# Psy-Fer/SquiggleKit

Measured on AMD Instinct MI355X. Metric: reads/sec MotifSeq DTW (4k-sample read x 200-sample motif), higher is better.
Workload: dtype f64 results; u32 fixed-point screening

## Files before the change

include/squigglekit_hip.h:

```cpp
#ifndef SQUIGGLEKIT_HIP_H
#define SQUIGGLEKIT_HIP_H

#include <stddef.h>
#include <stdint.h>

#ifdef __cplusplus
extern "C" {
#endif

typedef enum sk_status {
    SK_OK              =  0,
    SK_ERR_INVALID     = -1,
    SK_ERR_NO_DEVICE   = -2,
    SK_ERR_HIP         = -3,
    SK_ERR_NOMEM       = -4,
    SK_ERR_UNSUPPORTED = -5,
    SK_ERR_OVERFLOW    = -6
} sk_status;

enum { SK_SCALE_MEDMAD = 0, SK_SCALE_ZSCALE = 1 };

enum {
    SK_FLAG_EMPTY      = 1,
    SK_FLAG_DEGENERATE = 2,
// ... 338 lines not shown
    int32_t        kind;
    const void    *data;
    const int64_t *off;
} sk_fmt_col;
void *sk_fmt_rows(int64_t nrows, int32_t ncols, const sk_fmt_col *cols, const uint8_t *skip, int32_t nthreads,
                  int64_t *out_len);
void  sk_fmt_free(void *p);
void  sk_ndtr(const double *z, double *out, int64_t n);

int64_t sk_blow5_index(const void *buf, int64_t len, int64_t first, int64_t *rec_off, int64_t *rec_size, int64_t cap);
int64_t sk_blow5_index_some(const void *buf, int64_t len, int64_t pos, int64_t max_rec, int64_t *rec_off,
                            int64_t *rec_size, int64_t *next_pos);
int sk_blow5_rows_i16(const void *buf, int64_t len, const int64_t *rec_off, const int64_t *rec_size, int64_t nrec,
                      int32_t comp, int64_t stride, int16_t *rows, int32_t *nsamp, char *ids, int32_t id_width, double *calib,
                      int32_t *flags, int32_t nthreads);

int sk_comm_unique_id(void *id128);
int sk_comm_init_rank(const void *id128, int nranks, int rank);
int sk_comm_init_all(const int *devices, int ndev);
int sk_comm_info(int *nranks, int *rank);
int sk_comm_allgather_dev(const void *d_send, void *d_recv, size_t bytes);
int sk_comm_allgather_host(const void *send, void *recv, size_t bytes);
int sk_comm_destroy(void);

int sk_tunables(char *buf, int cap);

int sk_last_kernel_ms(float *prep_ms, float *main_ms);
int sk_last_dtw_retries(void);
int sk_last_dtw_tier2(void);
int sk_last_dtw_guard(int32_t *out );
int sk_last_dtw_premise_violations(void);
int sk_last_dtw_audit_mismatches(void);
int sk_last_dtw_window_steps(uint64_t *out );
int sk_last_f64_retries(void);
int sk_last_dtw_clock(double *ghz);
int sk_last_dtw_profile(float *dist_ms, int *dist_launches, float *start_ms, int *start_launches,
                        int *reads_per_launch);
int sk_synth_squiggles_dev(int16_t *d_sig, int64_t stride, int32_t nreads, int32_t nsamples,
                           uint64_t seed, const double *motif, int32_t nmotif);
typedef struct sk_synth_opts {
    int64_t        row0;
    int32_t        hit_permille;
    int32_t        stretch_permille;
    int32_t        stretch;
    const int16_t *tmpl;
    int32_t        ntmpl;
    double         tmpl_noise;
} sk_synth_opts;
int sk_synth_variant_dev(int16_t *d_sig, int64_t stride, int32_t nreads, int32_t nsamples, uint64_t seed,
                         const double *motif, int32_t nmotif, const sk_synth_opts *o);
int sk_synth_pa_dev(const int16_t *d_raw, int64_t stride, int32_t nreads, int32_t nsamples,
                    double offset, double range, double digitisation, double *d_out, int64_t *d_off);

typedef enum sk_pull_mode { SK_PULL_RAW = 0, SK_PULL_PA = 1 } sk_pull_mode;
int sk_pull_text(const int16_t *sig, int64_t stride, const int32_t *len, int32_t nreads, const double *calib, int32_t mode,
                 const char *prefix, const int64_t *prefix_off, char *text, int64_t capacity, int64_t *total,
                 int64_t *line_off);
int sk_pull_text_dev(const int16_t *d_sig, int64_t stride, const int32_t *d_len, int32_t nreads, const double *d_cal2,
                     int32_t mode, const char *d_prefix, const int64_t *d_prefix_off, char *d_text, int64_t capacity,
                     int64_t *total, int64_t *d_line_off);

typedef struct sk_det_params {
    int32_t w_short, w_long;
    double  th_short, th_long, peak_height;
} sk_det_params;
typedef struct sk_det_event {
// ... 73 lines not shown
```

squigglekit_amd/_lib.py:

```python
import ctypes as C
import os
import subprocess
import threading

import numpy as np

_HERE = os.path.dirname(os.path.abspath(__file__))
SO_PATH = os.environ.get("SK_LIB_PATH") or os.path.join(_HERE, "libsquigglekit_hip.so")
CSRC = os.path.join(_HERE, "csrc")


class SquiggleKitError(RuntimeError):
    def __init__(self, code, msg):
        super().__init__("squigglekit_hip error %d: %s" % (code, msg))
        self.code = code


SK_OK, SK_ERR_INVALID, SK_ERR_NO_DEVICE, SK_ERR_HIP, SK_ERR_NOMEM, SK_ERR_UNSUPPORTED, SK_ERR_OVERFLOW = 0, -1, -2, -3, -4, -5, -6
SK_SCALE = {"medmad": 0, "zscale": 1}
SK_PULL_RAW, SK_PULL_PA = 0, 1
SK_FLAG_EMPTY, SK_FLAG_DEGENERATE, SK_FLAG_RECENTRE = 1, 2, 4
SK_FLAG_CALIBRATING = 8
SK_STREAM_MAX_CALIB, SK_STREAM_MAX_SLOTS, SK_STREAM_MAX_POINTS = 65536, 65536, 1024

# ... 277 lines not shown
    "sk_dtw_subsequence_batch": (C.c_int, [_vp, C.c_int32, _vp, _vp, C.c_int32, _vp]),
    "sk_dtw_subsequence": (C.c_int, [_vp, C.c_int32, _vp, C.c_int32, _dp, _i32p, _i32p, _vp]),
    "sk_dtw_subsequence_cref": (C.c_int, [_vp, C.c_int32, _vp, C.c_int32, _dp, _i32p, _i32p]),
    "sk_normalise_i16": (C.c_int, [_vp, C.c_int32, C.c_int32, C.c_int32, C.c_int32, _vp, _i32p]),
    "sk_normalise_f64": (C.c_int, [_vp, C.c_int32, C.c_int32, C.c_int32, C.c_int32, _vp, _i32p]),
    "sk_tsv_count_lines": (C.c_int64, [_vp, C.c_size_t]),
    "sk_tsv_count_tokens": (C.c_int, [_vp, C.c_size_t, C.c_int32, C.c_int64, _vp, C.c_int32]),
    "sk_tsv_parse": (C.c_int, [_vp, C.c_size_t, C.c_int32, C.c_int64, _vp, _vp, _vp, _vp, _vp, _vp, _vp,
                               C.c_int32]),
    "sk_tsv_parse_centi": (C.c_int, [_vp, C.c_size_t, C.c_int32, C.c_int64, _vp, _vp, _vp, _vp, _vp, _vp, _vp,
                                     C.c_int32]),
    "sk_tsv_parse_i16": (C.c_int, [_vp, C.c_size_t, C.c_int32, C.c_int64, C.c_int64, _vp, _vp, _vp, _vp, _vp, _vp, _vp,
                                   _vp, C.c_int32]),
    "sk_fmt_rows": (_vp, [C.c_int64, C.c_int32, _vp, _vp, C.c_int32, _i64p]),
    "sk_fmt_free": (None, [_vp]),
    "sk_ndtr": (None, [_vp, _vp, C.c_int64]),
    "sk_blow5_index": (C.c_int64, [_vp, C.c_int64, C.c_int64, _vp, _vp, C.c_int64]),
    "sk_blow5_index_some": (C.c_int64, [_vp, C.c_int64, C.c_int64, C.c_int64, _vp, _vp, _vp]),
    "sk_blow5_rows_i16": (C.c_int, [_vp, C.c_int64, _vp, _vp, C.c_int64, C.c_int32, C.c_int64, _vp, _vp, _vp, C.c_int32, _vp, _vp,
                                    C.c_int32]),
    "sk_comm_unique_id": (C.c_int, [_vp]),
    "sk_comm_init_rank": (C.c_int, [_vp, C.c_int, C.c_int]),
    "sk_comm_init_all": (C.c_int, [_i32p, C.c_int]),
    "sk_comm_info": (C.c_int, [_i32p, _i32p]),
    "sk_comm_allgather_dev": (C.c_int, [_vp, _vp, C.c_size_t]),
    "sk_comm_allgather_host": (C.c_int, [_vp, _vp, C.c_size_t]),
    "sk_comm_destroy": (C.c_int, []),
    "sk_tunables": (C.c_int, [C.c_char_p, C.c_int]),
    "sk_last_kernel_ms": (C.c_int, [C.POINTER(C.c_float), C.POINTER(C.c_float)]),
    "sk_last_dtw_retries": (C.c_int, []),
    "sk_last_dtw_tier2": (C.c_int, []),
    "sk_last_dtw_guard": (C.c_int, [_i32p]),
    "sk_last_dtw_window_steps": (C.c_int, [_vp]),
    "sk_last_dtw_premise_violations": (C.c_int, []),
    "sk_last_dtw_audit_mismatches": (C.c_int, []),
    "sk_last_f64_retries": (C.c_int, []),
    "sk_last_dtw_clock": (C.c_int, [_dp]),
    "sk_last_dtw_profile": (C.c_int, [C.POINTER(C.c_float), _i32p, C.POINTER(C.c_float), _i32p, _i32p]),
    "sk_synth_squiggles_dev": (C.c_int, [_vp, C.c_int64, C.c_int32, C.c_int32, C.c_uint64, _vp, C.c_int32]),
    "sk_synth_variant_dev": (C.c_int, [_vp, C.c_int64, C.c_int32, C.c_int32, C.c_uint64, _vp, C.c_int32, _vp]),
    "sk_synth_pa_dev": (C.c_int, [_vp, C.c_int64, C.c_int32, C.c_int32, C.c_double, C.c_double, C.c_double, _vp, _vp]),
    "sk_pull_text": (C.c_int, [_vp, C.c_int64, _vp, C.c_int32, _vp, C.c_int32, _vp, _vp, _vp, C.c_int64, _i64p, _vp]),
    "sk_segment_sweep_i16": (C.c_int, [_vp, C.c_int64, _vp, C.c_int32, _vp, C.c_int32, _vp, _vp]),
    "sk_segment_sweep_dev_i16": (C.c_int, [_vp, C.c_int64, _vp, C.c_int32, _vp, C.c_int32, _vp, _vp]),
    "sk_segment_sweep_f64": (C.c_int, [_vp, _vp, _vp, C.c_int32, _vp, C.c_int32, _vp, _vp]),
    "sk_pull_text_dev": (C.c_int, [_vp, C.c_int64, _vp, C.c_int32, _vp, C.c_int32, _vp, _vp, _vp, C.c_int64, _i64p, _vp]),
    "sk_detect_events_i16": (C.c_int, [_vp, C.c_int64, _vp, C.c_int32, C.POINTER(DetParams), _vp, _vp, C.c_int64]),
    "sk_detect_events_dev_i16": (C.c_int, [_vp, C.c_int64, _vp, C.c_int32, C.POINTER(DetParams), _vp, _vp, C.c_int64]),
    "sk_hmm_viterbi_i16": (C.c_int, [_vp, C.c_int64, _vp, C.c_int32, _vp, C.POINTER(HmmModel), C.c_int32, _vp]),
    "sk_hmm_viterbi_dev_i16": (C.c_int, [_vp, C.c_int64, _vp, C.c_int32, _vp, C.POINTER(HmmModel), C.c_int32, _vp]),
    "sk_hmm_viterbi_f64_len": (C.c_int, [_vp, _vp, C.c_int32, C.POINTER(HmmModel), C.c_int32, _vp]),
    "sk_hmm_segments_i16": (C.c_int, [_vp, C.c_int64, _vp, C.c_int32, _vp, C.POINTER(HmmModel), C.c_int32, _vp, _vp, _vp,
                                      C.c_int64]),
    "sk_hmm_segments_dev_i16": (C.c_int, [_vp, C.c_int64, _vp, C.c_int32, _vp, C.POINTER(HmmModel), C.c_int32, _vp, _vp, _vp,
                                          C.c_int64]),
    "sk_hmm_segments_f64_len": (C.c_int, [_vp, _vp, C.c_int32, C.POINTER(HmmModel), C.c_int32, _vp, _vp, _vp, C.c_int64]),
    "sk_stream_open": (C.c_int, [_vp, _vp, C.c_int32, C.POINTER(StreamParams), _i32p]),
    "sk_stream_push_i16": (C.c_int, [C.c_int32, _vp, C.c_int32, _vp, C.c_int64, _vp, _vp]),
    "sk_stream_push_dev_i16": (C.c_int, [C.c_int32, _vp, C.c_int32, _vp, C.c_int64, _vp, _vp]),
    "sk_stream_flush": (C.c_int, [C.c_int32, _vp, C.c_int32, _vp]),
    "sk_stream_reset": (C.c_int, [C.c_int32, _vp, C.c_int32, _vp, _vp]),
    "sk_stream_close": (C.c_int, [C.c_int32]),
}


def build(force=False):
# ... 109 lines not shown
```

squigglekit_amd/csrc/sk_runtime.hip:

```cpp
#include "sk_common.h"
#include <string>
#include <string.h>
#include <mutex>
#include <stdio.h>
#include <stdlib.h>
#include <string.h>

static thread_local char  g_err[512] = "";
static thread_local int   g_cur = -1;
static sk_ctx             g_ctx[SK_MAX_DEVICES];
static std::mutex         g_mu;
static std::recursive_mutex g_ctx_mu[SK_MAX_DEVICES];

int sk_fail(int code, const char *fmt, ...)
{
    va_list ap;
    va_start(ap, fmt);
    vsnprintf(g_err, sizeof g_err, fmt, ap);
    va_end(ap);
    return code;
}

sk_entry::sk_entry() : sk_entry(g_cur) {}

// ... 16 lines not shown
sk_entry::~sk_entry() { if (c) g_ctx_mu[c - g_ctx].unlock(); }

sk_ctx *sk_ctx_of(int device) { return (device >= 0 && device < SK_MAX_DEVICES) ? &g_ctx[device] : nullptr; }
int sk_bound_device(void) { return g_cur; }

int sk_reserve(sk_ctx *c, sk_buf *b, size_t bytes)
{
    (void)c;
    if (bytes <= b->cap) return SK_OK;
    if (b->p) { SK_HIP(hipFree(b->p)); b->p = nullptr; b->cap = 0; }
    size_t want = bytes + bytes / 8 + 256;
    hipError_t e = hipMalloc(&b->p, want);
    if (e != hipSuccess) {
        b->p = nullptr;
        return sk_fail(SK_ERR_NOMEM, "hipMalloc(%zu) failed: %s", want, hipGetErrorString(e));
    }
    b->cap = want;
    return SK_OK;
}

int sk_second_stream(sk_ctx *c)
{
    if (!c->stream2) {
        SK_HIP(hipStreamCreateWithFlags(&c->stream2, hipStreamNonBlocking));
        for (int i = 0; i < 9; i++) SK_HIP(hipEventCreateWithFlags(&c->ev_chunk[i], hipEventDisableTiming));
    }
    return SK_OK;
}

struct sk_tunable { const char *name, *test_values, *what; };
static const sk_tunable SK_TUNABLES[] = {
    {"SK_DTW_SCHEME",         "full exact2", "DTW scheme: full = one exact pass, exact2 = two exact passes (default: fixed-point screening + certified window)"},
    {"SK_DTW_QL",             "8 16 64",     "lanes per read of the screening scheme (default: by motif length and batch size)"},
    {"SK_DTW_NOFUSE",         "1",           "filter + medmad as their own kernel instead of the screening pass's prologue"},
    {"SK_DTW_FORCE_RETRY_PM", "100 1000",    "per-mille of reads sent through the exact retry whatever the window pass certified (sensitivity runs)"},
    {"SK_DTW_SPAN",           "150 300",     "look-back of the window pass in columns (one tier)"},
    {"SK_DTW_SPAN2",          "0 500",       "look-back of the window pass's second tier (0: none)"},
    {"SK_DTW_CK",             "64 256",      "steps between checkpoints of the screening pass (multiple of 64)"},
    {"SK_DTW_NOSORT",         "1",           "window passes take the reads in file order"},
    {"SK_DTW_SORT_MIN",       "1",           "window passes sort chunks of at least this many reads"},
    {"SK_DTW_NO_EARLY",       "1",           "no early exact retry beside the window passes"},
    {"SK_DTW_NO_SIBLINGS",    "1",           "reads whose candidate columns fall into two clusters take the exact pass (no second window)"},
    {"SK_DTW_NOGUARD",        "1",           "screening scheme without its run-time guard (premise test in the window pass, audit, gated exact fallback): A/B cost runs"},
    {"SK_DTW_AUDIT_PERIOD",   "0 1 64",      "the audit re-runs one read in this many with the exact pass (default 4096; 0: no audit)"},
    {"SK_DTW_HOLE",           "qerr1 fma64 fma64x", "tests: a known precision hole put back (E = 1; the fma sample image for float64 reads, with / without the image-error guard) -- the guard has to notice and the records must not change"},
    {"SK_DTW_SCRATCH_MB",     "8 64",        "checkpoint scratch budget in MB (small values force many chunks)"},
    {"SK_DTW_NO_SMALL",       "1",           "small batches keep the batch lane layout"},
    {"SK_DTW_SMALL_MAX",      "0 100000",    "largest batch that spreads a read over 64 lanes"},
    {"SK_PREP_BLOCK",         "1",           "medmad statistics by the workgroup-per-read kernel"},
    {"SK_PREP_ROUNDS",        "1 3",         "grid rounds of the persistent statistics kernels"},
    {"SK_PREP_PERCU",         "1 2",         "workgroups per CU of the persistent statistics kernels"},
    {"SK_SEG_OLD",            "1",           "segmenter: numpy-order statistics kernels for every read"},
    {"SK_SEG_DELTA_SCALE",    "1e13",        "segmenter: certification margin multiplier (large: every read takes the numpy-order redo)"},
    {"SK_SEG_PA_F64",         "1",           "segmenter, raw reads through the pA conversion: expand to float64 and take the float64 kernels instead of the raw-domain kernel"},
    {"SK_SEG_NO_WG",          "1",           "segmenter, reads of 4 097 .. 65 536 samples: the wavefront-per-read statistics kernel (two looks at a read) instead of the workgroup-per-read one"},
    {"SK_SEG_WG_ALL",         "1",           "segmenter: the workgroup-per-read statistics kernel for every row of 4 097 .. 65 536 samples (default: where it is faster)"},
    {"SK_SEG_OCC",            "7 8",         "segmenter statistics kernel: waves per SIMD the registers are sized for"},
    {"SK_SEG_CHUNKS",         "2 8",         "segmenter: chunks of a large batch (walk of one beside the statistics of the next)"},
    {"SK_WALK_GENERAL",       "1",           "segmenter walk: general step (corrector test live)"},
    {"SK_WALK_SYNC",          "1",           "segmenter walk: run hopping with the 64 lanes of a wavefront on the same word (k_seg_walk3)"},
    {"SK_WALK_OWNPASS",       "1",           "segmenter walk: finds the quiet stretches and anchors in a pass of its own instead of taking the statistics kernel's hints"},
    {"SK_WALK_NOJUMP",        "1",           "segmenter walk: every run is hopped through, no jumps between the stretches of quiet entries"},
    {"SK_WALK_NOWAVE",        "1",           "segmenter walk: a lane per read also for long rows / small batches (no wavefront-per-read walk)"},
    {"SK_WALK_WAVE_MAXREADS", "0 1000000",   "segmenter walk: batches of up to this many reads take the wavefront-per-read walk (default: 16384, 131072 for rows beyond 4 096 samples)"},
    {"SK_DRNA_STEP",          "1",           "dRNA_segmenter, both branches: the per-sample scans instead of the scans by runs / by transitions"},
    {"SK_ROLL_TWO_KERNELS",   "1",           "dRNA_segmenter rolling-mean branch: filter kernel + prefix sums through HBM instead of the one-look kernel (prefix sums in LDS)"},
// ... 267 lines not shown
    if (!(c->retry_dev && c->dtwcnt.p)) return SK_OK;
    if (hipMemcpyAsync(out, (const int32_t *)c->dtwcnt.p + 8, 8 * sizeof(int32_t), hipMemcpyDeviceToHost, c->stream) != hipSuccess ||
        hipStreamSynchronize(c->stream) != hipSuccess)
        return sk_fail(SK_ERR_HIP, "reading the guard counters failed");
    return SK_OK;
}

int sk_last_dtw_premise_violations(void)
{
    int32_t g[8];
    const int rc = sk_last_dtw_guard(g);
    return rc ? rc : g[0];
}

int sk_last_dtw_audit_mismatches(void)
{
    int32_t g[8];
    const int rc = sk_last_dtw_guard(g);
    return rc ? rc : g[2];
}

int sk_last_dtw_window_steps(uint64_t *out)
{
    SK_ENTER(c);
    if (!out) return sk_fail(SK_ERR_INVALID, "NULL pointer");
    out[0] = out[1] = 0;
    if (!(c->retry_dev && c->dtwcnt.p && c->dtwcnt.cap >= 128)) return SK_OK;
    if (hipMemcpyAsync(out, (const char *)c->dtwcnt.p + 64, 16, hipMemcpyDeviceToHost, c->stream) != hipSuccess ||
        hipStreamSynchronize(c->stream) != hipSuccess)
        return sk_fail(SK_ERR_HIP, "reading the window-step counters failed");
    return SK_OK;
}

int sk_last_dtw_tier2(void)
{
    SK_ENTER(c);
    if (!(c->retry_dev && c->dtwcnt.p)) return 0;
    int32_t n = 0;
    if (hipMemcpyAsync(&n, (const int32_t *)c->dtwcnt.p + 1, sizeof n, hipMemcpyDeviceToHost, c->stream) != hipSuccess ||
        hipStreamSynchronize(c->stream) != hipSuccess)
        return sk_fail(SK_ERR_HIP, "reading the second-tier count failed");
    return n;
}

}
```

squigglekit_amd/csrc/sk_sdtwq.hip:

```cpp
#include "sk_sdtw_dev.h"
#include "sk_prepw_dev.h"
#include <math.h>
#include <stdlib.h>
#include <string.h>
#include <vector>

#ifndef SK_SDTWQ_FEED
#define SK_SDTWQ_FEED 0
#define SK_SDTWQ_MAIN 1
#endif

namespace {

template <int R>
__device__ __forceinline__ void qcolumn(const unsigned (&old)[R], unsigned (&nw)[R], const unsigned (&xq)[R],
                                        unsigned yq, unsigned dg, unsigned up)
{
    constexpr int R4 = R & ~3;
#pragma unroll
    for (int k = 0; k < R4; k += 4) {
        asm("v_min3_u32 %0, %12, %4, %13\n\t"
            "v_sad_u32 %0, %8, %14, %0 clamp\n\t"
            "v_min3_u32 %1, %4, %5, %0\n\t"
            "v_sad_u32 %1, %9, %14, %1 clamp\n\t"
            "v_min3_u32 %2, %5, %6, %1\n\t"
            "v_sad_u32 %2, %10, %14, %2 clamp\n\t"
            "v_min3_u32 %3, %6, %7, %2\n\t"
            "v_sad_u32 %3, %11, %14, %3 clamp"
            : "=&v"(nw[k]), "=&v"(nw[k + 1]), "=&v"(nw[k + 2]), "=&v"(nw[k + 3])
            : "v"(old[k]), "v"(old[k + 1]), "v"(old[k + 2]), "v"(old[k + 3]),
              "v"(xq[k]), "v"(xq[k + 1]), "v"(xq[k + 2]), "v"(xq[k + 3]),
              "v"(dg), "v"(up), "v"(yq));
        dg = old[k + 3];
        up = nw[k + 3];
    }
#pragma unroll
    for (int k = R4; k < R; k++) {
        asm("v_min3_u32 %0, %3, %1, %4\n\t"
            "v_sad_u32 %0, %2, %5, %0 clamp"
            : "=&v"(nw[k])
            : "v"(old[k]), "v"(xq[k]), "v"(dg), "v"(up), "v"(yq));
        dg = old[k];
        up = nw[k];
    }
}

__device__ __forceinline__ unsigned qimg(double v)
{
    return (unsigned)((int)rint(v * QSCALE)) + 0x80000000u;
}

template <int L>
__device__ __forceinline__ unsigned shr0(unsigned v, unsigned notfirst)
{
    if constexpr (L >= 16) {
        (void)notfirst;
        return (unsigned)__builtin_amdgcn_update_dpp(0, (int)v, (L == 16) ? DPP_ROW_SHR1 : DPP_WAVE_SHR1, 0xF, 0xF, true);
    } else {
        unsigned r;
        asm("s_nop 1\n\t"
            "v_and_b32_dpp %0, %1, %2 row_shr:1 row_mask:0xf bank_mask:0xf bound_ctrl:0"
            : "=v"(r) : "v"(v), "v"(notfirst));
        return r;
    }
}

struct wrec {
    int32_t tbase;
    int32_t jlo, jhi;
    int32_t flags;
};
struct sibrec {
    int32_t r;
    int32_t jlo, jhi;
    int32_t pad;
};

template <int L>
// ... 596 lines not shown
        const unsigned bq = (unsigned)a.qflag[r - a.read0];
        const double u = bestD * QSCALE, e = (double)a.qerr;
        const double e2 = (rec.flags & 4) ? 3.0 * e : e;
        const bool ok = fabs(u - (double)lq) <= e && u <= (double)bq + e2;
        if (!ok) { atomicAdd(&a.guard[SK_GUARD_VIOL], 1); atomicAdd(&a.guard[SK_GUARD_ALARM], 1); }
        return ok;
    };
    if (live && l == L - 1) {
        sk_hit h;
        h.n = n; h.flags = flags;
        const bool forced = a.force_retry && (((unsigned)r * 2654435761u) >> 22) < (unsigned)a.force_retry;
        bool certified = false;
        if (a.tier2 == 2) {
            h.dist = best; h.start = bestS; h.end = bestJ;
            h.n = (n > 0 && screened && bestS >= 0 && !forced && premise_holds(best, bestJ)) ? 1 : 0;
            a.sib_out[slot] = h;
        } else if (n <= 0) {
            h.dist = __builtin_nan(""); h.start = -1; h.end = -1;
            a.out[r] = h;
        } else if (screened && bestS >= 0 && !forced && (certified = premise_holds(best, bestJ))) {
            h.dist = best; h.start = bestS; h.end = bestJ;
            a.out[r] = h;
        } else if (!screened && a.early_cnt && !a.tier2) {
        } else {
            h.dist = __builtin_nan(""); h.start = -1; h.end = -1;
            a.out[r] = h;
            const bool violated = screened && bestS >= 0 && !forced && !certified;
            if (screened && a.soft && !forced && !violated) a.soft[atomicAdd(a.soft_cnt, 1)] = r;
            else                                            a.retry[atomicAdd(a.retry_cnt, 1)] = r;
        }
    }
}

typedef void (*sdtw_fn)(const sdtw_kargs);

template <int L, int FEED, int WHICH>
sdtw_fn pick_r(int R)
{
#define SK_KERNEL(RR) (WHICH == 0 ? (sdtw_fn)k_sdtw_q<L, RR, FEED, false> :     \
                       WHICH == 3 ? (sdtw_fn)k_sdtw_q<L, RR, FEED, (RR >= 2)> : \
                       WHICH == 1 ? (sdtw_fn)k_sdtw_p<L, RR, FEED> : (sdtw_fn)k_sdtw_w<L, RR, FEED>)
    switch (R) { SK_R_CASES_1_16(SK_KERNEL) }
    if constexpr (L != 64) {
        switch (R) { SK_R_CASES_17_32(SK_KERNEL) }
    }
#undef SK_KERNEL
    return nullptr;
}

template <int WHICH, int FEED>
sdtw_fn pick_l(int L, int R)
{
    if (L == 8)  return pick_r<8, FEED, WHICH>(R);
    if (L == 16) return pick_r<16, FEED, WHICH>(R);
    return pick_r<64, FEED, WHICH>(R);
}

}

#if SK_SDTWQ_FEED == 0
void *sk_sdtwq_pick_feed0(int which, int L, int R)
#elif SK_SDTWQ_FEED == 1
void *sk_sdtwq_pick_feed1(int which, int L, int R)
#else
void *sk_sdtwq_pick_feed2(int which, int L, int R)
#endif
{
    switch (which) {
    case 0: return (void *)pick_l<0, SK_SDTWQ_FEED>(L, R);
    case 1: return (void *)pick_l<1, SK_SDTWQ_FEED>(L, R);
    case 3: return (void *)pick_l<3, SK_SDTWQ_FEED>(L, R);
    default: return (void *)pick_l<2, SK_SDTWQ_FEED>(L, R);
    }
}

#ifdef SK_SDTWQ_MAIN
void *sk_sdtwq_pick_feed1(int which, int L, int R);
void *sk_sdtwq_pick_feed2(int which, int L, int R);

static void screen_layout(int N, int64_t nreads, int64_t maxlen, int *L, int *R)
{
    int l = (N <= 8 * 32 && nreads >= (maxlen > 8192 ? 65536 : 49152)) ? 8 : (N <= 16 * 32) ? 16 : 64;
    if (const char *e = sk_tune("SK_DTW_QL")) {
        const int v = atoi(e);
        if ((v == 8 && N <= 8 * 32) || (v == 16 && N <= 16 * 32) || v == 64) l = v;
    }
    *L = l;
    *R = (N + l - 1) / l;
}

constexpr int ORDER_BINS = 1024;

struct order_args {
    const wrec    *rec;
    const int32_t *qflag;
    int nreads, read0, span, ck, nck, L, wmax;
    int32_t *hist;
    int32_t *order;
};

__device__ __forceinline__ int order_key(const order_args &a, int i)
{
    const wrec q = a.rec[i];
    const unsigned b = (unsigned)a.qflag[i];
// ... 117 lines not shown
    int64_t chunk;
    while (true) {
        chunk = sk_dtw_chunk_reads(per_read, a->nreads);
        rc = sk_reserve(c, &c->ckpt, (size_t)chunk * (size_t)(nck > 0 ? nck : 1) * ck_bytes);
        if (!rc) rc = sk_reserve(c, &c->lastq, (size_t)chunk * lq_stride * sizeof(unsigned));
        if (!rc) rc = sk_reserve(c, &c->wstate, (size_t)chunk * state_bytes);
        if (!rc) rc = sk_reserve(c, &c->lsum, (size_t)chunk * (size_t)(nck + 1) * L * sizeof(unsigned));
        if (rc != SK_ERR_NOMEM || chunk <= 1024) break;
        sk_dtw_scratch_shrink(0);
    }
    if (rc) return rc;
    if ((rc = sk_reserve(c, &c->qflag, (size_t)chunk * sizeof(int32_t)))) return rc;
    if ((rc = sk_reserve(c, &c->wrec, (size_t)chunk * sizeof(wrec)))) return rc;
    if ((rc = sk_reserve(c, &c->wrecq, (size_t)chunk * sizeof(wrec)))) return rc;
    int sort_min = 32768;
    if (const char *e = sk_tune("SK_DTW_SORT_MIN")) { const int v = atoi(e); if (v > 0) sort_min = v; }
    const bool sorted = chunk >= sort_min && sk_tune("SK_DTW_NOSORT") == nullptr;
    if (sorted && (rc = sk_reserve(c, &c->order, ((size_t)chunk + ORDER_BINS) * sizeof(int32_t)))) return rc;
    const bool tiers = span2 > span;
    if (tiers && (rc = sk_reserve(c, &c->wsoft, ((size_t)chunk + 1) * sizeof(int32_t)))) return rc;
    const bool siblings = sk_tune("SK_DTW_NO_SIBLINGS") == nullptr;
    const int sib_cap = (int)(chunk / 64 + 1024);
    if (siblings) {
        if ((rc = sk_reserve(c, &c->sib, 16 + (size_t)sib_cap * sizeof(sibrec)))) return rc;
        if ((rc = sk_reserve(c, &c->sibout, (size_t)sib_cap * sizeof(sk_hit)))) return rc;
        if ((rc = sk_reserve(c, &c->sibstate, (size_t)sib_cap * (state_bytes + sizeof(wrec))))) return rc;
        if (c->stream3 && !c->ev_s[0])
            for (int i = 0; i < 2; i++) SK_HIP(hipEventCreateWithFlags(&c->ev_s[i], hipEventDisableTiming));
    }

    typedef void *(*pick_fn)(int, int, int);
    const pick_fn pk = a->feed == SK_FEED_I16 ? (pick_fn)sk_sdtwq_pick_feed0
                     : a->feed == SK_FEED_F64_NORM ? (pick_fn)sk_sdtwq_pick_feed1 : (pick_fn)sk_sdtwq_pick_feed2;
    sdtw_fn fq = (sdtw_fn)pk(P == 0 ? 3 : 0, L, R), fp = (sdtw_fn)pk(1, L, R), fw = (sdtw_fn)pk(2, L, R);
    if (!fq || !fp || !fw) return sk_fail(SK_ERR_UNSUPPORTED, "no screening kernel for L=%d R=%d", L, R);

    sdtw_kargs k = kargs_of(a);
    k.xlay = (const double *)c->motifw.p; k.xlayq = (const unsigned *)c->motifq.p; k.P = P; k.out = a->out;
    k.nck = nck; k.ck = ck; k.span = span; k.retry = d_retry; k.retry_cnt = d_retry_cnt;
    k.ckq = (unsigned *)c->ckpt.p; k.lastq = (unsigned *)c->lastq.p; k.lq_stride = (int64_t)lq_stride;
    k.qflag = (int32_t *)c->qflag.p; k.lsum = (unsigned *)c->lsum.p;
    k.wstate = (unsigned *)c->wstate.p; k.wrec = c->wrec.p; k.wrec_q = c->wrecq.p;
    k.early_cnt = d_early_cnt; k.early = d_early;
    k.qerr = (unsigned)(N + maxlen + 2);
    k.wmax = 4 * ck;
    k.lds_wave_words = (64 / L) * ck;
    k.guard = sk_tune("SK_DTW_NOGUARD") ? nullptr : (int32_t *)c->dtwcnt.p + 8;
    k.wsteps = (unsigned long long *)((char *)c->dtwcnt.p + 64);
    if (const char *e = sk_tune("SK_DTW_HOLE")) {
        k.hole = strcmp(e, "qerr1") == 0 ? SK_HOLE_QERR1 : strcmp(e, "fma64") == 0 ? SK_HOLE_FMA64
               : strcmp(e, "fma64x") == 0 ? SK_HOLE_FMA64_UNGUARDED : SK_HOLE_NONE;
        if (k.hole == SK_HOLE_QERR1) k.qerr = 1;
    }
    if (const char *e = sk_tune("SK_DTW_FORCE_RETRY_PM")) {
        const int pm = atoi(e);
        if (pm > 0) k.force_retry = pm >= 1000 ? 1024 : (pm * 1024 + 999) / 1000;
    }

    size_t fz_lds = 0;
    const sk_prep_fuse fz = a->fuse ? *a->fuse : sk_prep_fuse();
    if (a->fuse) {
        const int need = fz.mode == SK_PREP_ZSCALE ? (int)((a->stride * 2 + 15) / 16 * 4) : (((fz.hi - fz.lo - 1) + 3) & ~3);
        if (need > k.lds_wave_words) k.lds_wave_words = need;
    }
    fz_lds = (size_t)4 * (size_t)k.lds_wave_words * sizeof(unsigned);
    if (fz_lds + 5 * 1024 > 64 * 1024)
        return sk_fail(SK_ERR_INVALID, "SK_DTW_CK=%d with %d lanes per read needs %zu bytes of LDS per workgroup (limit 65536): "
// ... 97 lines not shown
```

Measured before the change: 16.82 million.

## Add hand-scheduled inline-asm window DTW kernel with LDS motif prefetch ring

Adds k_sdtw_wl, a new default exact window-pass kernel whose DTW cell update is written as interleaved inline GCN assembly (two cells in flight, f64 min/compare/cndmask for the start index). For R>16 it keeps the motif in LDS and software-prefetches the next four values with ds_read into a ring buffer while the current group computes. The intent is to beat the compiler's schedule on the serial dependency chain and cut register pressure. The old C++ kernel stays reachable through SK_DTW_WCELL=c, and a debug accessor for window records is added. Hand-written asm plus manual lgkmcnt waits risk hazards and make the code harder to maintain.

```diff
diff --git a/include/squigglekit_hip.h b/include/squigglekit_hip.h
--- a/include/squigglekit_hip.h
+++ b/include/squigglekit_hip.h
@@ -394,6 +394,7 @@
 int sk_last_dtw_premise_violations(void);
 int sk_last_dtw_audit_mismatches(void);
 int sk_last_dtw_window_steps(uint64_t *out );
+int sk_last_dtw_windows(int32_t *out , int nslots);
 int sk_last_f64_retries(void);
 int sk_last_dtw_clock(double *ghz);
 int sk_last_dtw_profile(float *dist_ms, int *dist_launches, float *start_ms, int *start_launches,
diff --git a/squigglekit_amd/_lib.py b/squigglekit_amd/_lib.py
--- a/squigglekit_amd/_lib.py
+++ b/squigglekit_amd/_lib.py
@@ -333,6 +333,7 @@
     "sk_last_dtw_tier2": (C.c_int, []),
     "sk_last_dtw_guard": (C.c_int, [_i32p]),
     "sk_last_dtw_window_steps": (C.c_int, [_vp]),
+    "sk_last_dtw_windows": (C.c_int, [_vp, C.c_int]),
     "sk_last_dtw_premise_violations": (C.c_int, []),
     "sk_last_dtw_audit_mismatches": (C.c_int, []),
     "sk_last_f64_retries": (C.c_int, []),
diff --git a/squigglekit_amd/csrc/sk_runtime.hip b/squigglekit_amd/csrc/sk_runtime.hip
--- a/squigglekit_amd/csrc/sk_runtime.hip
+++ b/squigglekit_amd/csrc/sk_runtime.hip
@@ -72,6 +72,7 @@
 static const sk_tunable SK_TUNABLES[] = {
     {"SK_DTW_SCHEME",         "full exact2", "DTW scheme: full = one exact pass, exact2 = two exact passes (default: fixed-point screening + certified window)"},
     {"SK_DTW_QL",             "8 16 64",     "lanes per read of the screening scheme (default: by motif length and batch size)"},
+    {"SK_DTW_WCELL",          "c",           "exact window pass with the cell as the compiler schedules it from C++ (k_sdtw_w) instead of the laid-out one (k_sdtw_wl)"},
     {"SK_DTW_NOFUSE",         "1",           "filter + medmad as their own kernel instead of the screening pass's prologue"},
     {"SK_DTW_FORCE_RETRY_PM", "100 1000",    "per-mille of reads sent through the exact retry whatever the window pass certified (sensitivity runs)"},
     {"SK_DTW_SPAN",           "150 300",     "look-back of the window pass in columns (one tier)"},
@@ -405,6 +406,19 @@
     return SK_OK;
 }
 
+int sk_last_dtw_windows(int32_t *out, int nslots)
+{
+    SK_ENTER(c);
+    if (!out || nslots < 0) return sk_fail(SK_ERR_INVALID, "NULL pointer or negative count");
+    const size_t bytes = (size_t)nslots * 4 * sizeof(int32_t);
+    if (!c->wrec.p || c->wrec.cap < bytes) return sk_fail(SK_ERR_INVALID, "no window records for %d slots", nslots);
+    if (bytes == 0) return SK_OK;
+    if (hipMemcpyAsync(out, c->wrec.p, bytes, hipMemcpyDeviceToHost, c->stream) != hipSuccess ||
+        hipStreamSynchronize(c->stream) != hipSuccess)
+        return sk_fail(SK_ERR_HIP, "reading the window records failed");
+    return SK_OK;
+}
+
 int sk_last_dtw_tier2(void)
 {
     SK_ENTER(c);
diff --git a/squigglekit_amd/csrc/sk_sdtwq.hip b/squigglekit_amd/csrc/sk_sdtwq.hip
--- a/squigglekit_amd/csrc/sk_sdtwq.hip
+++ b/squigglekit_amd/csrc/sk_sdtwq.hip
@@ -44,6 +44,131 @@
         up = nw[k];
     }
 }
+
+#define SK_W_A(m, c, t, dk, dkm1, sk, skm1, xk)                 \
+    "v_cmp_lt_f64 vcc, " dk ", " dkm1 "\n\t"                    \
+    "v_min_f64 " m ", " dk ", " dkm1 "\n\t"                     \
+    "v_add_f64 " c ", " xk ", -%[y]\n\t"                        \
+    "v_cndmask_b32 " t ", " skm1 ", " sk ", vcc\n\t"
+#define SK_W_B(m, c, t, dk, sk, u, us)                          \
+    "v_cmp_lt_f64 vcc, " u ", " m "\n\t"                        \
+    "v_min_f64 " m ", " u ", " m "\n\t"                         \
+    "v_add_f64 " dk ", |" c "|, " m "\n\t"                      \
+    "v_cndmask_b32 " sk ", " t ", " us ", vcc\n\t"
+#define SK_W_FOUR                                                                           \
+    SK_W_A("%[mb]", "%[cb]", "%[tb]", "%[d1]", "%[d0]", "%[s1]", "%[s0]", "%[x1]")          \
+    SK_W_B("%[m]", "%[c]", "%[t]", "%[d0]", "%[s0]", "%[u]", "%[us]")                       \
+    SK_W_A("%[m]", "%[c]", "%[t]", "%[d2]", "%[d1]", "%[s2]", "%[s1]", "%[x2]")             \
+    SK_W_B("%[mb]", "%[cb]", "%[tb]", "%[d1]", "%[s1]", "%[d0]", "%[s0]")                   \
+    SK_W_A("%[mb]", "%[cb]", "%[tb]", "%[d3]", "%[d2]", "%[s3]", "%[s2]", "%[x3]")          \
+    SK_W_B("%[m]", "%[c]", "%[t]", "%[d2]", "%[s2]", "%[d1]", "%[s1]")                      \
+    SK_W_A("%[m]", "%[c]", "%[t]", "%[d4]", "%[d3]", "%[s4]", "%[s3]", "%[x4]")             \
+    SK_W_B("%[mb]", "%[cb]", "%[tb]", "%[d3]", "%[s3]", "%[d2]", "%[s2]")
+#define SK_W_FOUR_OUT                                                                                   \
+    [d0] "+v"(D[k]), [d1] "+v"(D[k + 1]), [d2] "+v"(D[k + 2]), [d3] "+v"(D[k + 3]),                     \
+    [s0] "+v"(S[k]), [s1] "+v"(S[k + 1]), [s2] "+v"(S[k + 2]), [s3] "+v"(S[k + 3]),                     \
+    [m] "+v"(m), [c] "+v"(c), [t] "+v"(t), [mb] "=&v"(mb), [cb] "=&v"(cb), [tb] "=&v"(tb)
+#define SK_W_FETCH                                  \
+    "ds_read_b64 %[n0], %[xa] offset:%[o0]\n\t"     \
+    "ds_read_b64 %[n1], %[xa] offset:%[o1]\n\t"     \
+    "ds_read_b64 %[n2], %[xa] offset:%[o2]\n\t"     \
+    "ds_read_b64 %[n3], %[xa] offset:%[o3]\n\t"
+struct wring_of {
+    int R;
+    constexpr int groups() const { return (R - 1 + 3) / 4; }
+    constexpr int buf(int j) const { return (j == groups() - 1 && (groups() & 1)) ? 2 : (j & 1); }
+    constexpr int off(int j, int i) const { return 8 * (4 * j + 1 + i < R ? 4 * j + 1 + i : R - 1); }
+};
+template <int R>
+__device__ __forceinline__ void wring_prime(double (&xb)[3][4], unsigned xa)
+{
+    constexpr wring_of w{R};
+    asm volatile(SK_W_FETCH
+                 : [n0] "=&v"(xb[0][0]), [n1] "=&v"(xb[0][1]), [n2] "=&v"(xb[0][2]), [n3] "=&v"(xb[0][3])
+                 : [xa] "v"(xa), [o0] "n"(w.off(0, 0)), [o1] "n"(w.off(0, 1)), [o2] "n"(w.off(0, 2)), [o3] "n"(w.off(0, 3)));
+}
+__device__ __forceinline__ void wring_drain(double (&xb)[3][4])
+{
+    asm volatile("s_waitcnt lgkmcnt(0)" : "+v"(xb[0][0]), "+v"(xb[0][1]), "+v"(xb[0][2]), "+v"(xb[0][3]));
+}
+template <int R, bool XLDS>
+__device__ __forceinline__ void wcolumn(double (&D)[R], int (&S)[R], const double (&xr)[XLDS ? 1 : R], double x0,
+                                        double (&xb)[3][4], unsigned xa, double y,
+                                        double dgD, int dgS, double upD, int upS)
+{
+    constexpr wring_of w{R};
+    double m, c, mb, cb;
+    int t, tb;
+    asm(SK_W_A("%[m]", "%[c]", "%[t]", "%[d0]", "%[dg]", "%[s0]", "%[sg]", "%[x0]")
+        : [m] "=&v"(m), [c] "=&v"(c), [t] "=&v"(t)
+        : [d0] "v"(D[0]), [dg] "v"(dgD), [s0] "v"(S[0]), [sg] "v"(dgS), [x0] "v"(x0), [y] "v"(y)
+        : "vcc");
+    constexpr int R4 = (R - 1) & ~3;
+#pragma unroll
+    for (int k = 0; k < R4; k += 4) {
+        const double u = k ? D[k - 1] : upD;
+        const int us = k ? S[k - 1] : upS;
+        if constexpr (XLDS) {
+            constexpr int NG = w.groups();
+            const int j = k / 4, jn = (j + 1) % NG;
+            double (&cur)[4] = xb[w.buf(j)];
+            double (&nxt)[4] = xb[w.buf(jn)];
+            asm volatile("s_waitcnt lgkmcnt(0)\n\t"
+                SK_W_FETCH
+                SK_W_FOUR
+                : SK_W_FOUR_OUT, [n0] "=&v"(nxt[0]), [n1] "=&v"(nxt[1]), [n2] "=&v"(nxt[2]), [n3] "=&v"(nxt[3])
+                : [d4] "v"(D[k + 4]), [s4] "v"(S[k + 4]),
+                  [x1] "v"(cur[0]), [x2] "v"(cur[1]), [x3] "v"(cur[2]), [x4] "v"(cur[3]),
+                  [y] "v"(y), [u] "v"(u), [us] "v"(us), [xa] "v"(xa),
+                  [o0] "n"(w.off(jn, 0)), [o1] "n"(w.off(jn, 1)), [o2] "n"(w.off(jn, 2)), [o3] "n"(w.off(jn, 3))
+                : "vcc");
+        } else {
+            asm(SK_W_FOUR
+                : SK_W_FOUR_OUT
+                : [d4] "v"(D[k + 4]), [s4] "v"(S[k + 4]),
+                  [x1] "v"(xr[k + 1]), [x2] "v"(xr[k + 2]), [x3] "v"(xr[k + 3]), [x4] "v"(xr[k + 4]),
+                  [y] "v"(y), [u] "v"(u), [us] "v"(us)
+                : "vcc");
+        }
+    }
+    if constexpr (XLDS && R4 < R - 1) {
+        constexpr int NG = w.groups();
+        double (&cur)[4] = xb[w.buf(NG - 1)];
+        double (&nxt)[4] = xb[0];
+        asm volatile("s_waitcnt lgkmcnt(0)\n\t"
+            SK_W_FETCH
+            : "+v"(cur[0]), "+v"(cur[1]), "+v"(cur[2]), "+v"(cur[3]),
+              [n0] "=&v"(nxt[0]), [n1] "=&v"(nxt[1]), [n2] "=&v"(nxt[2]), [n3] "=&v"(nxt[3])
+            : [xa] "v"(xa), [o0] "n"(w.off(0, 0)), [o1] "n"(w.off(0, 1)), [o2] "n"(w.off(0, 2)), [o3] "n"(w.off(0, 3)));
+    }
+#pragma unroll
+    for (int k = R4; k < R; k++) {
+        const double u = k ? D[k - 1] : upD;
+        const int us = k ? S[k - 1] : upS;
+        if (k + 1 < R) {
+            double x1;
+            if constexpr (XLDS) x1 = xb[w.buf(w.groups() - 1)][k - R4];
+            else                x1 = xr[k + 1];
+            asm(SK_W_A("%[mb]", "%[cb]", "%[tb]", "%[d1]", "%[d0]", "%[s1]", "%[s0]", "%[x1]")
+                SK_W_B("%[m]", "%[c]", "%[t]", "%[d0]", "%[s0]", "%[u]", "%[us]")
+                : [d0] "+v"(D[k]), [s0] "+v"(S[k]), [m] "+v"(m), [mb] "=&v"(mb), [cb] "=&v"(cb), [tb] "=&v"(tb)
+                : [d1] "v"(D[k + 1]), [s1] "v"(S[k + 1]), [x1] "v"(x1), [y] "v"(y), [u] "v"(u), [us] "v"(us),
+                  [c] "v"(c), [t] "v"(t)
+                : "vcc");
+            m = mb; c = cb; t = tb;
+        } else {
+            asm(SK_W_B("%[m]", "%[c]", "%[t]", "%[d0]", "%[s0]", "%[u]", "%[us]")
+                : [d0] "+v"(D[k]), [s0] "+v"(S[k]), [m] "+v"(m)
+                : [u] "v"(u), [us] "v"(us), [c] "v"(c), [t] "v"(t)
+                : "vcc");
+        }
+    }
+}
+#undef SK_W_FOUR
+#undef SK_W_FOUR_OUT
+#undef SK_W_FETCH
+#undef SK_W_A
+#undef SK_W_B
 
 __device__ __forceinline__ unsigned qimg(double v)
 {
@@ -706,6 +831,217 @@
     }
 }
 
+template <int L, int R, int FEED>
+__global__ __launch_bounds__(256) __attribute__((amdgpu_waves_per_eu(R <= 13 ? 4 : (R <= 26 ? 3 : 2), 8)))
+void k_sdtw_wl(const sdtw_kargs a)
+{
+    constexpr int G = 64 / L;
+    constexpr bool XLDS = R > 16;
+    constexpr int SHR = (L == 64) ? DPP_WAVE_SHR1 : DPP_ROW_SHR1;
+    constexpr int CKW = R + 2;
+    constexpr int U = XLDS ? 4 : 8;
+    const double INF = __builtin_huge_val();
+
+    const int lane = threadIdx.x & 63;
+    const int wave = blockIdx.x * (blockDim.x >> 6) + (threadIdx.x >> 6);
+    const int g = lane / L, l = lane % L;
+    int slot = wave * G + g;
+    int nreads = a.nreads;
+    if (a.wl_count) {
+        nreads = min(*a.wl_count, a.nreads);
+        if (nreads <= 0) return;
+    }
+    const bool live = slot < nreads;
+    if (!live) slot = nreads - 1;
+    const int r = a.tier2 == 2 ? ((const sibrec *)a.sib)[slot].r : a.wl_list ? a.wl_list[slot] : a.read0 + slot;
+
+    int n, flags = 0;
+    double center = 0.0, scale = 1.0;
+    const int16_t *s16 = nullptr;
+    const double  *s64 = nullptr;
+    if constexpr (FEED == SK_FEED_I16) {
+        const sk_prep pr = a.prep[r];
+        n = pr.n; flags = pr.flags & SK_FLAG_PUBLIC; center = pr.center; scale = pr.scale;
+        s16 = (const int16_t *)a.samples + (int64_t)r * a.stride;
+    } else if constexpr (FEED == SK_FEED_F64_NORM) {
+        const sk_prep pr = a.prep[r];
+        n = pr.n; flags = pr.flags & SK_FLAG_PUBLIC; center = pr.center; scale = pr.scale;
+        s64 = (const double *)(((pr.flags & SK_IFLAG_INPLACE) && a.samples_raw) ? a.samples_raw : a.samples) + a.off[r];
+    } else {
+        n = (int)(a.off[r + 1] - a.off[r]);
+        if (n == 0) flags = SK_FLAG_EMPTY;
+        s64 = (const double *)a.samples + a.off[r];
+    }
+    if (!live) n = 0;
+
+    const wrec rec = ((const wrec *)a.wrec)[slot];
+    const bool screened = live && (rec.flags & 1);
+    const bool restored = screened && (rec.flags & 2);
+    const int tbase = screened ? rec.tbase : 0;
+    const int jlo = rec.jlo, jhi = rec.jhi;
+    const int tlast = screened ? jhi + L - 1 : -1;
+    const bool shortlane = l < a.P;
+    const unsigned notfirst = (l == 0) ? 0u : 0xffffffffu;
+    const unsigned first = ~notfirst;
+
+    int nsteps = tlast - tbase + 1;
+    if (nsteps < 0) nsteps = 0;
+    const int own_steps = nsteps;
+#pragma unroll
+    for (int d = L; d < 64; d <<= 1) nsteps = max(nsteps, __shfl_xor(nsteps, d));
+    nsteps = __builtin_amdgcn_readfirstlane(nsteps);
+    const int nblk = (nsteps + L - 1) / L;
+    if (a.wsteps) {
+        __shared__ unsigned long long lds_steps[2];
+        int own_sum = live ? own_steps : 0;
+#pragma unroll
+        for (int d = L; d < 64; d <<= 1) own_sum += __shfl_xor(own_sum, d);
+        if (threadIdx.x == 0) { lds_steps[0] = 0; lds_steps[1] = 0; }
+        __syncthreads();
+        if (lane == 0) {
+            atomicAdd(&lds_steps[0], (unsigned long long)(nblk * L));
+            atomicAdd(&lds_steps[1], (unsigned long long)own_sum);
+        }
+        __syncthreads();
+        if (threadIdx.x == 0) {
+            if (lds_steps[0]) atomicAdd(&a.wsteps[0], lds_steps[0]);
+            if (lds_steps[1]) atomicAdd(&a.wsteps[1], lds_steps[1]);
+        }
+    }
+
+    double x[XLDS ? 1 : R];
+    constexpr int RP = R | 1;
+    __shared__ double lds_x[XLDS ? L * RP : 1];
+    if constexpr (XLDS) {
+        for (int i = threadIdx.x; i < L * R; i += blockDim.x) lds_x[(i / R) * RP + i % R] = a.xlay[i];
+        __syncthreads();
+    } else {
+#pragma unroll
+        for (int k = 0; k < R; k++) x[k] = a.xlay[l * R + k];
+    }
+    typedef __attribute__((address_space(3))) const double lds_row;
+    const unsigned xa = XLDS ? (unsigned)(size_t)(lds_row *)(lds_x + l * RP) : 0u;
+    const double x0 = XLDS ? lds_x[l * RP] : x[0];
+    double xb[3][4];
+    if constexpr (XLDS) wring_prime<R>(xb, xa);
+
+    const int nlast = max(n - 1, 0);
+    if (n == 0) { s16 = (const int16_t *)a.xlay; s64 = (const double *)a.xlay; }
+    auto fetch = [&](int idx) -> double {
+        const int ci = min(max(idx, 0), nlast);
+        double v;
+        if constexpr (FEED == SK_FEED_I16)           v = ((double)s16[ci] - center) / scale;
+        else if constexpr (FEED == SK_FEED_F64_NORM) v = (s64[ci] - center) / scale;
+        else                                         v = s64[ci];
+        return (idx < 0 || idx >= n) ? INF : v;
+    };
+    auto lb = [&](unsigned q) -> double { return (double)(q > a.qerr ? q - a.qerr : 0u) * QUNIT; };
+
+    double D[R];
+    int    S[R];
+#pragma unroll
+    for (int k = 0; k < R; k++) { D[k] = INF; S[k] = -1; }
+    double botD = (R == 1 && l == 0 && shortlane) ? 0.0 : INF;
+    int    botS = (R == 1 && l == 0 && shortlane) ? 0 : -1;
+    double diagD = (l == 0) ? 0.0 : INF;
+    int    diagS = (l == 0) ? tbase : -1;
+    if (restored) {
+        const unsigned *ws = a.wstate + ((int64_t)slot * L + l) * CKW;
+#pragma unroll
+        for (int k = 0; k < R; k++) D[k] = lb(ws[k]);
+        botD = lb(ws[R]);
+        if (l > 0) diagD = lb(ws[R + 1]);
+        if (R == 1 && l == 0 && shortlane) { botD = 0.0; botS = tbase; }
+    }
+    double best = INF;  int bestS = -1, bestJ = -1;
+    int s0 = screened ? max(jlo - tbase + L - 1, 0) : 0x7fffffff;
+#pragma unroll
+    for (int d = L; d < 64; d <<= 1) s0 = min(s0, __shfl_xor(s0, d));
+    s0 = __builtin_amdgcn_readfirstlane(s0);
+
+    __shared__ double lds_w[4][3 * 64];
+    double *ybuf = lds_w[threadIdx.x >> 6] + g * 3 * L;
+    ybuf[L + l] = fetch(tbase - L + l);
+    double F = fetch(tbase + l);
+    for (int blk = 0; blk < nblk; blk++) {
+        const double Fnext = fetch(tbase + (blk + 1) * L + l);
+        const double *yr;
+        if (blk & 1) { ybuf[L + l] = F; yr = ybuf + L - l; }
+        else         { ybuf[l] = F; ybuf[2 * L + l] = F; yr = ybuf + 2 * L - l; }
+#pragma unroll 1
+        for (int qq = 0; qq < L; qq += U) {
+            double yv[U];
+#pragma unroll
+            for (int q = 0; q < U; q++) yv[q] = yr[qq + q];
+#pragma unroll
+            for (int q = 0; q < U; q++) {
+                const int t = tbase + blk * L + qq + q;
+                const double y = yv[q];
+                double upD;  int upS;
+                if constexpr (L >= 16) {
+                    upD = dpp_f64<SHR>(0.0, botD);
+                    upS = dpp_i32<SHR>(t + 1, botS);
+                } else {
+                    const unsigned lo = shr0<L>((unsigned)__double2loint(botD), notfirst);
+                    const unsigned hi = shr0<L>((unsigned)__double2hiint(botD), notfirst);
+                    upD = __hiloint2double((int)hi, (int)lo);
+                    upS = (int)(shr0<L>((unsigned)botS, notfirst) | (first & (unsigned)(t + 1)));
+                }
+                wcolumn<R, XLDS>(D, S, x, x0, xb, xa, y, diagD, diagS, upD, upS);
+                diagD = upD;  diagS = upS;
+                if constexpr (R >= 2) {
+                    botD = shortlane ? D[R - 2] : D[R - 1];
+                    botS = shortlane ? S[R - 2] : S[R - 1];
+                } else {
+                    botD = shortlane ? upD : D[0];
+                    botS = shortlane ? upS : S[0];
+                }
+                if (blk * L + qq + q >= s0) {
+                    const int j = t - l;
+                    if (j >= jlo && j <= jhi && D[R - 1] < best) { best = D[R - 1]; bestS = S[R - 1]; bestJ = j; }
+                }
+            }
+        }
+        F = Fnext;
+    }
+    if constexpr (XLDS) wring_drain(xb);
+
+    auto premise_holds = [&](double bestD, int j) -> bool {
+        if (!a.guard) return true;
+        const unsigned lq = a.lastq[(int64_t)(r - a.read0) * a.lq_stride + j + L];
+        const unsigned bq = (unsigned)a.qflag[r - a.read0];
+        const double u = bestD * QSCALE, e = (double)a.qerr;
+        const double e2 = (rec.flags & 4) ? 3.0 * e : e;
+        const bool ok = fabs(u - (double)lq) <= e && u <= (double)bq + e2;
+        if (!ok) { atomicAdd(&a.guard[SK_GUARD_VIOL], 1); atomicAdd(&a.guard[SK_GUARD_ALARM], 1); }
+        return ok;
+    };
+    if (live && l == L - 1) {
+        sk_hit h;
+        h.n = n; h.flags = flags;
+        const bool forced = a.force_retry && (((unsigned)r * 2654435761u) >> 22) < (unsigned)a.force_retry;
+        bool certified = false;
+        if (a.tier2 == 2) {
+            h.dist = best; h.start = bestS; h.end = bestJ;
+            h.n = (n > 0 && screened && bestS >= 0 && !forced && premise_holds(best, bestJ)) ? 1 : 0;
+            a.sib_out[slot] = h;
+        } else if (n <= 0) {
+            h.dist = __builtin_nan(""); h.start = -1; h.end = -1;
+            a.out[r] = h;
+        } else if (screened && bestS >= 0 && !forced && (certified = premise_holds(best, bestJ))) {
+            h.dist = best; h.start = bestS; h.end = bestJ;
+            a.out[r] = h;
+        } else if (!screened && a.early_cnt && !a.tier2) {
+        } else {
+            h.dist = __builtin_nan(""); h.start = -1; h.end = -1;
+            a.out[r] = h;
+            const bool violated = screened && bestS >= 0 && !forced && !certified;
+            if (screened && a.soft && !forced && !violated) a.soft[atomicAdd(a.soft_cnt, 1)] = r;
+            else                                            a.retry[atomicAdd(a.retry_cnt, 1)] = r;
+        }
+    }
+}
+
 typedef void (*sdtw_fn)(const sdtw_kargs);
 
 template <int L, int FEED, int WHICH>
@@ -713,7 +1049,8 @@
 {
 #define SK_KERNEL(RR) (WHICH == 0 ? (sdtw_fn)k_sdtw_q<L, RR, FEED, false> :     \
                        WHICH == 3 ? (sdtw_fn)k_sdtw_q<L, RR, FEED, (RR >= 2)> : \
-                       WHICH == 1 ? (sdtw_fn)k_sdtw_p<L, RR, FEED> : (sdtw_fn)k_sdtw_w<L, RR, FEED>)
+                       WHICH == 1 ? (sdtw_fn)k_sdtw_p<L, RR, FEED> :             \
+                       WHICH == 4 ? (sdtw_fn)k_sdtw_w<L, RR, FEED> : (sdtw_fn)k_sdtw_wl<L, RR, FEED>)
     switch (R) { SK_R_CASES_1_16(SK_KERNEL) }
     if constexpr (L != 64) {
         switch (R) { SK_R_CASES_17_32(SK_KERNEL) }
@@ -744,6 +1081,7 @@
     case 0: return (void *)pick_l<0, SK_SDTWQ_FEED>(L, R);
     case 1: return (void *)pick_l<1, SK_SDTWQ_FEED>(L, R);
     case 3: return (void *)pick_l<3, SK_SDTWQ_FEED>(L, R);
+    case 4: return (void *)pick_l<4, SK_SDTWQ_FEED>(L, R);
     default: return (void *)pick_l<2, SK_SDTWQ_FEED>(L, R);
     }
 }
@@ -927,7 +1265,9 @@
     typedef void *(*pick_fn)(int, int, int);
     const pick_fn pk = a->feed == SK_FEED_I16 ? (pick_fn)sk_sdtwq_pick_feed0
                      : a->feed == SK_FEED_F64_NORM ? (pick_fn)sk_sdtwq_pick_feed1 : (pick_fn)sk_sdtwq_pick_feed2;
-    sdtw_fn fq = (sdtw_fn)pk(P == 0 ? 3 : 0, L, R), fp = (sdtw_fn)pk(1, L, R), fw = (sdtw_fn)pk(2, L, R);
+    sdtw_fn fq = (sdtw_fn)pk(P == 0 ? 3 : 0, L, R), fp = (sdtw_fn)pk(1, L, R);
+    const char *wcell = sk_tune("SK_DTW_WCELL");
+    sdtw_fn fw = (sdtw_fn)pk(wcell && strcmp(wcell, "c") == 0 ? 4 : 2, L, R);
     if (!fq || !fp || !fw) return sk_fail(SK_ERR_UNSUPPORTED, "no screening kernel for L=%d R=%d", L, R);
 
     sdtw_kargs k = kargs_of(a);
```

New measurement: 16.89 million (median of 6 runs). No clear change (+0.4%).
